# winlaic/ZipVoice

Hardware: AMD Instinct MI355X
Metric: generated mel-frames/s (whole job) + RTF, ZipVoice 123M N_steps=16 batch=32/GPU (higher is better)
Workload: dtype bf16; 1 GPU; C2: ZipVoice 123M, N_steps=16, batch=32/GPU x (3 s prompt + 10 s generated; T=1219 frames), CFG g=1.0 (64 decoder rows per GPU), t_shift=0.5; model=zipvoice (zipvoice_base.json, synthetic seeded weights), global_batch=32, seq_len=1219, parallelism=dp1

## Files before the change

### zipvoice_amd/csrc/zv_ffn.inc

```
#pragma once
#include <cstddef>
#include "zv_gemm256.inc"
#include "zv_weights.inc"

typedef unsigned v4u32_t __attribute__((ext_vector_type(4)));
typedef unsigned v2u32_t __attribute__((ext_vector_type(2)));
constexpr int FFN_D = 512, FFN_BM = 128, FFN_HC = 32, FFN_SLOT = 32768, FFN_MAXSEG = 4;
constexpr long FFN_PART_FLOATS = (long)FFN_BM * FFN_D;

struct FfnSeg {
  int M, rb0;
  const bf16* X;
  const bf16* A;
  const float* resid; float* C;
  bf16* Ch;
  const float* rowvec;
  const float* orig;
  bf16* Cl; bf16* C2h; bf16* C2l;
};

struct FfnParams {
  int H;
  int R, nseg;
  FfnSeg seg[FFN_MAXSEG];
  long ldx, ldc, ldch, rowvec_ld; int rows_per_group;
  const bf16* W1f; const float* b1;
  const bf16* W2f; const float* b2;
  const float* byp;
  const bf16* Wpf; const float* bp; long lda; int nkp;
  const float* nb; float log_scale;
  float norm_scale;
  float* sink;
  int w;
  float* part; unsigned* flag; int part_slots;
  unsigned* err;
  unsigned long long* dbg;
};

#ifndef FFN_NORM_LDS
#define FFN_NORM_LDS 1
#endif
#ifndef FFN_XOVL
#define FFN_XOVL 1
#endif
constexpr int FFN_NCONST = 3 * FFN_D + 4 * 2 * FFN_D;
inline size_t ffn_lds_bytes(int H, bool norm = false) {
  return 4 * FFN_SLOT + ((size_t)H + FFN_HC) * 4 +
         (norm && FFN_NORM_LDS ? FFN_NCONST * 4 : 0);
}

#ifdef ZV_OPERAND_F16
#define FFN_MFMA "v_mfma_f32_32x32x16_f16"
#else
#define FFN_MFMA "v_mfma_f32_32x32x16_bf16"
#endif
#ifndef FFN_BIAS_ACC
#define FFN_BIAS_ACC 1
#endif
__device__ __forceinline__ void ffn_mma_v0(f32x16& acc, const bf16x8& a, const bf16x8& b) {
  asm volatile(FFN_MFMA " %0, %1, %2, 0" : "=&v"(acc) : "v"(a), "v"(b));
}
__device__ __forceinline__ void ffn_mma_v(f32x16& acc, const bf16x8& a, const bf16x8& b) {
  asm volatile(FFN_MFMA " %0, %1, %2, %0" : "+v"(acc) : "v"(a), "v"(b));
}
#ifndef FFN_OUT_ASM
#define FFN_OUT_ASM 1
#endif
__device__ __forceinline__ void ffn_mma_a(f32x16& acc, const bf16x8& a, const bf16x8& b) {
#if FFN_OUT_ASM
  asm volatile(FFN_MFMA " %0, %1, %2, %0" : "+a"(acc) : "v"(a), "v"(b));
#else
  acc = ZV_MFMA_32x32x16(a, b, acc, 0, 0, 0);
#endif
}
struct FfnAct { float t, m, q; };
__device__ __forceinline__ void ffn_act_op(int sub, float& y, FfnAct& a, float b, float c0, float cq) {
  if (sub == 0) {
#if FFN_BIAS_ACC
    asm volatile("v_fmamk_f32 %0, %1, 0x3fb8aa3b, %2" : "=&v"(a.t) : "v"(y), "v"(c0));
#else
    asm volatile("v_add_f32 %0, %0, %2\n\tv_fmamk_f32 %1, %0, 0x3fb8aa3b, %3" : "+&v"(y), "=&v"(a.t) : "v"(b), "v"(c0));
#endif
  } else if (sub == 1) {
    asm volatile("v_min_f32 %0, 0x42fc0000, %1\n\tv_exp_f32 %0, %0" : "=&v"(a.m) : "v"(a.t));
  } else if (sub == 2) {
    asm volatile("v_add_f32 %0, 1.0, %0\n\tv_log_f32 %0, %0" : "+v"(a.m));
  } else {
    asm volatile("v_fmamk_f32 %1, %0, 0xbda3d70a, %4\n\tv_max_f32 %2, %2, %3\n\tv_fmamk_f32 %0, %2, 0x3f317218, %1"
                 : "+&v"(y), "=&v"(a.q), "+&v"(a.m) : "v"(a.t), "v"(cq));
  }
}

#ifndef FFN_DMA_K0
#define FFN_DMA_K0 1
#define FFN_DMA_K1 17
#define FFN_DMA_K2 33
#define FFN_DMA_K3 49
#endif
#ifndef FFN_TIMING
#define FFN_TIMING 0
#endif
#ifndef FFN_PD
#define FFN_PD 12
#endif
#ifndef FFN_PD_OPRE
#define FFN_PD_OPRE 8
#endif
#ifndef FFN_PD_NORM
#define FFN_PD_NORM 16
#endif
constexpr int FFN_DBG_WORDS = 10;
#ifndef FFN_X_NOACT
#define FFN_X_NOACT 0
#endif
#ifndef FFN_X_NOW1
#define FFN_X_NOW1 0
#endif
#ifndef FFN_X_NOW2
#define FFN_X_NOW2 0
#endif
#ifndef FFN_EPI_T
#define FFN_EPI_T 1
#endif
#ifndef FFN_PT
#define FFN_PT 16
#endif
#ifndef FFN_EPI_NT
#define FFN_EPI_NT 1
#endif
#ifndef FFN_PT_NORM
#define FFN_PT_NORM 8
#endif
constexpr unsigned long long FFN_SPIN_TICKS = 200000000;

template <bool RV, bool ORIG, bool COPY, int ABL = 0, int NORM = 0, bool TP = true, bool PRE = false>
__global__ __launch_bounds__(256, 1) void zv_ffn_kernel(FfnParams p) {
  extern __shared__ __attribute__((aligned(16))) unsigned char smem[];
  const int tid = threadIdx.x, lane = tid & 63;
  const int wave = __builtin_amdgcn_readfirstlane(tid >> 6);
  const int tl = lane & 31, hh = lane >> 5;
  const int nc = p.H / FFN_HC;
  float* b1s = reinterpret_cast<float*>(smem + 4 * FFN_SLOT);
  const long Wtot = (long)p.R * nc;
  const long start = (long)blockIdx.x * p.w;
  if (start >= Wtot) return;
  const long end = min(start + (long)p.w, Wtot);

  auto dma = [&](const bf16* W, int c, int slot, int half) {
    const unsigned long long a = (unsigned long long)W + (unsigned long long)((long)c * FFN_SLOT + wave * 8192 + half * 4096);
    const unsigned long long b =
        ((unsigned long long)(unsigned)__builtin_amdgcn_readfirstlane((unsigned)(a >> 32)) << 32) |
        (unsigned long long)(unsigned)__builtin_amdgcn_readfirstlane((unsigned)a);
    glds16s_x4(reinterpret_cast<const void*>(b), (unsigned)lane * 16u, smem + slot * FFN_SLOT + wave * 8192 + half * 4096);
  };
  auto item_at = [&](long ps, int& r, int& ca, int& cb) {
    r = (int)(ps / nc);
    const int c = (int)(ps - (long)r * nc);
    if (c != 0) { ca = 0; cb = nc - c; }
    else if (ps + nc <= end) { ca = 0; cb = nc; }
    else { ca = nc - (int)(end - ps); cb = nc; }
  };

  int r, ca, cb;
  item_at(start, r, ca, cb);
  dma(p.W1f, ca, 0, 0); dma(p.W1f, ca, 0, 1);
  dma(p.W1f, ca + 1, 1, 0); dma(p.W1f, ca + 1, 1, 1);
  for (int i = tid; i < p.H + FFN_HC; i += 256) b1s[i] = i < p.H ? p.b1[i] : 0.f;
  constexpr bool NLDS = NORM && FFN_NORM_LDS;
  float* ncs = b1s + p.H + FFN_HC;
  if constexpr (NLDS) {
    for (int i = tid; i < FFN_D; i += 256) {
      ncs[i] = p.b2[i];
      ncs[FFN_D + i] = p.nb[i];
      ncs[2 * FFN_D + i] = p.byp[i];
    }
  }

  float c0 = -5.77078016355585362f, cq = -0.035f;
  asm volatile("" : "+v"(c0), "+v"(cq));
  const int lfrag = lane * 16;
  int lfrag2 = lane * 16 + 2 * FFN_SLOT;
  asm volatile("" : "+v"(lfrag2));
  auto w1f = [&](int sl, int s) { return *reinterpret_cast<const bf16x8*>(smem + sl * FFN_SLOT + s * 1024 + lfrag); };
  auto w2f = [&](int sl, int i) { return *reinterpret_cast<const bf16x8*>(smem + sl * FFN_SLOT + i * 1024 + lfrag2); };
  auto put = [&](bf16x8 (&hb)[2], int rr, float y) { hb[rr >> 3][rr & 7] = (bf16)y; };
  const __amdgpu_buffer_rsrc_t part_rs = __builtin_amdgcn_make_buffer_rsrc(p.part, 0, 0x7fffffff, 0x00020000);

#if FFN_TIMING
  unsigned long long tm_vm = 0, tm_bar = 0, tm_steps = 0, tm_epi = 0, tm_x = 0, tm_items = 0, tm_loop = 0;
  const unsigned long long tm_t0 = __builtin_amdgcn_s_memtime(), tm_r0 = __builtin_amdgcn_s_memrealtime();
#endif
  auto item = [&](auto KIND_, int r, int ca, int cb, bool has_next, int nca) {
    constexpr int KIND = decltype(KIND_)::value;
    constexpr bool split_in = KIND == 2, split_out = KIND == 1;
    const int nxt_c0 = has_next ? nca : cb - 1;
    const int nxt_c1 = has_next ? nca + 1 : cb - 1;
    f32x16 out[16];
    int sg = 0;
#pragma unroll
    for (int i = 1; i < FFN_MAXSEG; ++i) sg = (i < p.nseg && r >= p.seg[i].rb0) ? i : sg;
    typedef __attribute__((address_space(4))) const FfnSeg KSeg;
    KSeg& S = ((KSeg*)((__attribute__((address_space(4))) const char*)__builtin_amdgcn_kernarg_segment_ptr() +
                       offsetof(FfnParams, seg)))[sg];
    const int t0 = (r - S.rb0) * FFN_BM + wave * 32;

    if constexpr (split_in) {
      if (tid == 0) {
        GLOBAL unsigned* fl = (GLOBAL unsigned*)(p.flag + blockIdx.x + 1);
        const unsigned long long t_give_up = wall_clock64() + FFN_SPIN_TICKS;
        while (__hip_atomic_load(fl, __ATOMIC_RELAXED, __HIP_MEMORY_SCOPE_AGENT) == 0u) {
          __builtin_amdgcn_s_sleep(2);
          if (wall_clock64() > t_give_up) {
            if (p.err) __hip_atomic_store(p.err, 1u, __ATOMIC_RELAXED, __HIP_MEMORY_SCOPE_SYSTEM);
            break;
          }
        }
        __builtin_amdgcn_fence(__ATOMIC_ACQUIRE, "agent");
        __hip_atomic_store(fl, 0u, __ATOMIC_RELAXED, __HIP_MEMORY_SCOPE_AGENT);
      }
      asm volatile("s_waitcnt vmcnt(0)" ::: "memory");
      __syncthreads();
      int lv = lane;
      asm volatile("" : "+v"(lv));
      const f32x4* src = reinterpret_cast<const f32x4*>(p.part + (long)(blockIdx.x + 1) * FFN_PART_FLOATS) + wave * 4096 + lv;
      static_for<16>([&](auto J_) {
        constexpr int j = decltype(J_)::value;
        f32x4 v[4];
#pragma unroll
        for (int q = 0; q < 4; ++q) v[q] = src[(j * 4 + q) * 64];
        out[j] = f32x16{v[0][0], v[0][1], v[0][2], v[0][3], v[1][0], v[1][1], v[1][2], v[1][3],
                        v[2][0], v[2][1], v[2][2], v[2][3], v[3][0], v[3][1], v[3][2], v[3][3]};
        __builtin_amdgcn_sched_barrier(0);
      });
    } else if constexpr (!PRE) {
#pragma unroll
      for (int j = 0; j < 16; ++j) out[j] = f32x16{};
    }
    if constexpr (!PRE || split_in) {
#pragma unroll
      for (int j = 0; j < 16; ++j) asm volatile("" : "+a"(out[j]));
    }
#if FFN_TIMING
    const unsigned long long tx0 = __builtin_amdgcn_s_memtime();
    ++tm_items;
#endif
    const bool nrv = NLDS && !split_out && S.rowvec != nullptr && p.rows_per_group >= 32;
    const int nrv_g0 = nrv ? min(t0, S.M - 1) / p.rows_per_group : 0;
    f32x4 nrvv[4];
    if constexpr (NLDS && !split_out) {
      if (nrv) {
        const int g1 = min(nrv_g0 + 1, (S.M - 1) / p.rows_per_group);
#pragma unroll
        for (int q = 0; q < 4; ++q) {
          const int f = (q * 64 + lane) * 4;
          const int grp = f < FFN_D ? nrv_g0 : g1;
          nrvv[q] = *reinterpret_cast<const f32x4*>(S.rowvec + (long)grp * p.rowvec_ld + (f & (FFN_D - 1)));
        }
      }
    }
    bf16x8 xf[32];
    if constexpr (!PRE) {
      const int tr = min(t0 + tl, S.M - 1);
      const bf16* xr = S.X + (long)tr * p.ldx + 8 * hh;
#pragma unroll
      for (int s = 0; s < 32; ++s) xf[s] = *reinterpret_cast<const bf16x8*>(xr + 16 * s);
    } else if constexpr (split_in) {
      const int tr = min(t0 + tl, S.M - 1);
      const bf16* xr = S.Ch + (long)tr * p.ldch + 4 * hh;
#pragma unroll
      for (int s = 0; s < 32; ++s) {
        const bf16x4 lo = *reinterpret_cast<const bf16x4*>(xr + 16 * s), hi = *reinterpret_cast<const bf16x4*>(xr + 16 * s + 8);
        xf[s] = bf16x8{lo[0], lo[1], lo[2], lo[3], hi[0], hi[1], hi[2], hi[3]};
      }
    }
    wait_vmcnt<(FFN_XOVL && !PRE) ? 32 : 0>();
    if constexpr (NLDS && !split_out) {
      if (nrv) {
#pragma unroll
        for (int q = 0; q < 4; ++q)
          *reinterpret_cast<f32x4*>(ncs + 3 * FFN_D + wave * 2 * FFN_D + (q * 64 + lane) * 4) = nrvv[q];
      }
    }
    __syncthreads();
#if FFN_TIMING
    tm_x += __builtin_amdgcn_s_memtime() - tx0;
#endif

    if constexpr (PRE && !split_in) {
      int lvp = lane;
      asm volatile("" : "+v"(lvp));
      const int ptl = lvp & 31, phh = lvp >> 5;
      const int wr = max(0, min(32, S.M - t0));
      const __amdgpu_buffer_rsrc_t rs_a =
          __builtin_amdgcn_make_buffer_rsrc(const_cast<bf16*>(S.A + (long)t0 * p.lda), 0, wr * (int)p.lda * 2, 0x00020000);
      const __amdgpu_buffer_rsrc_t rs_pr =
          __builtin_amdgcn_make_buffer_rsrc(const_cast<float*>(S.resid + (long)t0 * p.ldc), 0, wr * (int)p.ldc * 4, 0x00020000);
      const int a_off = (ptl * (int)p.lda + 8 * phh) * 2, r_off = (ptl * (int)p.ldc + 4 * phh) * 4;
      auto load_a = [&](int kc, int s) {
        return __builtin_bit_cast(bf16x8, __builtin_amdgcn_raw_buffer_load_b128(rs_a, a_off + kc * 64 + s * 32, 0, 0));
      };
      dma(p.Wpf, 0, 2, 0); dma(p.Wpf, 0, 2, 1);
      bf16x8 ac[2], an[2];
      ac[0] = load_a(0, 0); ac[1] = load_a(0, 1);
      const bool hrv = S.rowvec != nullptr;
      const int rpg = hrv ? p.rows_per_group : 1;
      auto tile_of = [&](const f32x4 (&v)[4]) {
        return f32x16{v[0][0], v[0][1], v[0][2], v[0][3], v[1][0], v[1][1], v[1][2], v[1][3],
                      v[2][0], v[2][1], v[2][2], v[2][3], v[3][0], v[3][1], v[3][2], v[3][3]};
      };
      if (!hrv || rpg >= 32) {
        float* cvs = reinterpret_cast<float*>(smem + 3 * FFN_SLOT) + wave * 2 * FFN_D;
        const int g0 = hrv ? min(t0, S.M - 1) / rpg : 0;
        const int g1 = hrv ? min(g0 + 1, (S.M - 1) / rpg) : 0;
#pragma unroll
        for (int q = 0; q < 4; ++q) {
          const int f = (q * 64 + lvp) * 4, ch = f & (FFN_D - 1);
          f32x4 v = *reinterpret_cast<const f32x4*>(p.bp + ch);
          if (hrv) v += *reinterpret_cast<const f32x4*>(S.rowvec + (long)(f < FFN_D ? g0 : g1) * p.rowvec_ld + ch);
          *reinterpret_cast<f32x4*>(cvs + f) = v;
        }
        asm volatile("s_waitcnt lgkmcnt(0)" ::: "memory");
        __builtin_amdgcn_wave_barrier();
        const float* cvp = cvs + ((hrv && t0 + ptl >= (g0 + 1) * rpg) ? FFN_D : 0) + 4 * phh;
        constexpr int PDT = 6;
        f32x4 ri[16][4];
        auto pf = [&](int j) {
          if (j < 16) {
#pragma unroll
            for (int q = 0; q < 4; ++q)
              ri[j][q] = __builtin_bit_cast(f32x4, __builtin_amdgcn_raw_buffer_load_b128(rs_pr, r_off + (32 * j + 8 * q) * 4, 0, 0));
          }
        };
#pragma unroll
        for (int j = 0; j < PDT; ++j) pf(j);
        static_for<16>([&](auto J_) {
          constexpr int j = decltype(J_)::value;
          pf(j + PDT);
          f32x4 v[4];
#pragma unroll
          for (int q = 0; q < 4; ++q) v[q] = ri[j][q] + *reinterpret_cast<const f32x4*>(cvp + 32 * j + 8 * q);
          out[j] = tile_of(v);
          asm volatile("" : "+a"(out[j]));
          __builtin_amdgcn_sched_barrier(0);
        });
      } else {
        const int grp = min(t0 + ptl, S.M - 1) / rpg;
        const float* vrow = S.rowvec + (long)grp * p.rowvec_ld + 4 * phh;
        const float* bpl = p.bp + 4 * phh;
        static_for<16>([&](auto J_) {
          constexpr int j = decltype(J_)::value;
          f32x4 v[4];
#pragma unroll
          for (int q = 0; q < 4; ++q) {
            const f32x4 r4 = __builtin_bit_cast(f32x4, __builtin_amdgcn_raw_buffer_load_b128(rs_pr, r_off + (32 * j + 8 * q) * 4, 0, 0));
            v[q] = r4 + (*reinterpret_cast<const f32x4*>(bpl + 32 * j + 8 * q) + *reinterpret_cast<const f32x4*>(vrow + 32 * j + 8 * q));
          }
          out[j] = tile_of(v);
          asm volatile("" : "+a"(out[j]));
          if constexpr ((j & 3) == 3) __builtin_amdgcn_sched_barrier(0);
        });
      }
      auto pstep = [&](auto PAR_, int kc) {
        constexpr int PAR = decltype(PAR_)::value;
        wait_vmcnt<0>();
        asm volatile("s_waitcnt lgkmcnt(0)" ::: "memory");
        __builtin_amdgcn_s_barrier();
        asm volatile("s_nop 7\n\ts_nop 7\n\ts_nop 3" ::: "memory");
        if (kc + 1 < p.nkp) { dma(p.Wpf, kc + 1, 3 - PAR, 0); dma(p.Wpf, kc + 1, 3 - PAR, 1); }
        const int kn = min(kc + 1, p.nkp - 1);
        an[0] = load_a(kn, 0); an[1] = load_a(kn, 1);
        bf16x8 fb[4];
#pragma unroll
        for (int q = 0; q < 4; ++q) fb[q] = w2f(PAR, q);
        static_for<32>([&](auto I_) {
          constexpr int i = decltype(I_)::value;
          ffn_mma_a(out[i >> 1], fb[i & 3], ac[i & 1]);
          if constexpr (i + 4 < 32) fb[i & 3] = w2f(PAR, i + 4);
        });
        asm volatile("" ::"v"(ac[0]), "v"(ac[1]), "v"(fb[0]), "v"(fb[1]), "v"(fb[2]), "v"(fb[3]));
        ac[0] = an[0]; ac[1] = an[1];
      };
      int kc = 0;
      for (; kc + 1 < p.nkp; kc += 2) {
        pstep(std::integral_constant<int, 0>{}, kc);
        pstep(std::integral_constant<int, 1>{}, kc + 1);
      }
      if (kc < p.nkp) pstep(std::integral_constant<int, 0>{}, kc);
      asm volatile("s_nop 7\n\ts_nop 7\n\ts_nop 3" ::: "memory");
#pragma unroll
      for (int j = 0; j < 16; ++j) asm volatile("" : "+a"(out[j]));
      static_for<32>([&](auto S_) {
        constexpr int s = decltype(S_)::value, jt = s >> 1, pp = s & 1;
#pragma unroll
        for (int e = 0; e < 8; ++e) xf[s][e] = (bf16)out[jt][8 * pp + e];
      });
#pragma unroll
      for (int j = 0; j < 16; ++j) asm volatile("" : "+a"(out[j]));
      if constexpr (split_out) {
        const __amdgpu_buffer_rsrc_t rs_xh =
            __builtin_amdgcn_make_buffer_rsrc(S.Ch + (long)t0 * p.ldch, 0, wr * (int)p.ldch * 2, 0x00020000);
        const int h_off = (ptl * (int)p.ldch + 4 * phh) * 2;
        static_for<32>([&](auto S_) {
          constexpr int s = decltype(S_)::value;
          const v4u32_t w = __builtin_bit_cast(v4u32_t, xf[s]);
          __builtin_amdgcn_raw_buffer_store_b64(v2u32_t{w[0], w[1]}, rs_xh, h_off + 32 * s, 0, 16);
          __builtin_amdgcn_raw_buffer_store_b64(v2u32_t{w[2], w[3]}, rs_xh, h_off + 32 * s + 16, 0, 16);
        });
      }
#pragma unroll
      for (int s = 0; s < 32; ++s) asm volatile("" : "+v"(xf[s]));
      asm volatile("s_nop 7\n\ts_nop 7\n\ts_nop 3" ::: "memory");
    }

    auto bias4 = [&](int c, int q) { return *reinterpret_cast<const f32x4*>(b1s + c * FFN_HC + 8 * q + 4 * hh); };
    auto bias_tile = [&](int c) {
      const f32x4 q0 = bias4(c, 0), q1 = bias4(c, 1), q2 = bias4(c, 2), q3 = bias4(c, 3);
      return f32x16{q0[0], q0[1], q0[2], q0[3], q1[0], q1[1], q1[2], q1[3],
                    q2[0], q2[1], q2[2], q2[3], q3[0], q3[1], q3[2], q3[3]};
    };
    f32x16 h0, h1;
#if FFN_BIAS_ACC
    h0 = bias_tile(ca);
    h1 = bias_tile(ca + 1);
#endif
    {
      bf16x8 f[4];
#pragma unroll
      for (int q = 0; q < 4; ++q) f[q] = w1f(0, q);
      static_for<32>([&](auto S_) {
        constexpr int s = decltype(S_)::value;
        if constexpr (s == 0 && !FFN_BIAS_ACC) ffn_mma_v0(h0, f[0], xf[0]);
        else ffn_mma_v(h0, f[s & 3], xf[s]);
        if constexpr (s + 4 < 32) f[s & 3] = w1f(0, s + 4);
      });
    }
    asm volatile("s_nop 7\n\ts_nop 7\n\ts_nop 3" : "+v"(h0));
    __builtin_amdgcn_s_barrier();

    auto sync = [&]() {
#if FFN_TIMING
      const unsigned long long ts0 = __builtin_amdgcn_s_memtime();
#endif
      wait_vmcnt<0>();
      asm volatile("s_waitcnt lgkmcnt(0)" ::: "memory");
#if FFN_TIMING
      const unsigned long long ts1 = __builtin_amdgcn_s_memtime();
#endif
      __builtin_amdgcn_s_barrier();
#if FFN_TIMING
      const unsigned long long ts2 = __builtin_amdgcn_s_memtime();
      tm_vm += ts1 - ts0;
      tm_bar += ts2 - ts1;
      ++tm_steps;
#endif
      asm volatile("s_nop 7\n\ts_nop 7\n\ts_nop 3" ::: "memory");
    };
    auto w1_next = [&](int c) { return c + 2 <= cb - 1 ? c + 2 : (c + 2 == cb ? nxt_c0 : nxt_c1); };

    bf16x8 hb0[2], hb1[2];
    {
      const int c1 = w1_next(ca);
      dma(p.W1f, c1, 0, 0); dma(p.W1f, c1, 0, 1);
      dma(p.W2f, ca, 2, 0); dma(p.W2f, ca, 2, 1);
      f32x4 bq = FFN_BIAS_ACC ? f32x4{} : bias4(ca, 0);
      FfnAct a{};
      bf16x8 f[4];
#pragma unroll
      for (int q = 0; q < 4; ++q) f[q] = w1f(1, q);
      static_for<32>([&](auto S_) {
        constexpr int s = decltype(S_)::value, rr = s >> 1;
        if constexpr (s == 0 && !FFN_BIAS_ACC) ffn_mma_v0(h1, f[0], xf[0]);
        else ffn_mma_v(h1, f[s & 3], xf[s]);
        if constexpr (s + 4 < 32) f[s & 3] = w1f(1, s + 4);
        if constexpr ((rr & 3) == 0 && (s & 1) == 0 && !FFN_BIAS_ACC) bq = bias4(ca, rr >> 2);
        float y = h0[rr];
        ffn_act_op(2 * (s & 1), y, a, bq[rr & 3], c0, cq);
        ffn_act_op(2 * (s & 1) + 1, y, a, bq[rr & 3], c0, cq);
        h0[rr] = y;
        if constexpr (s & 1) put(hb0, rr, y);
      });
#if FFN_BIAS_ACC
      h0 = bias_tile(min(ca + 2, nc));
#endif
      asm volatile("s_nop 7\n\ts_nop 7\n\ts_nop 3" : "+v"(h1));
      sync();
      asm volatile("" ::"v"(f[0]), "v"(f[1]), "v"(f[2]), "v"(f[3]));
    }

    const int m = t0 + tl;
    const bool row_ok = m < S.M;
    const long mr = min(m, S.M - 1);
    const float* rrow = S.resid + mr * p.ldc;
    const float* orow = (ORIG || NORM) ? S.orig + mr * p.ldc : nullptr;
    constexpr bool OPRE = ORIG && !NORM;
    constexpr int PD = NORM ? FFN_PD_NORM : OPRE ? FFN_PD_OPRE : FFN_PD;
    f32x4 rr[32][2], ro[OPRE ? 32 : 1][2];
    auto prefetch = [&](int g) {
      if (g < 32) {
        const int n = 16 * g + 8 * hh;
        if constexpr (!PRE) {
          rr[g][0] = *reinterpret_cast<const f32x4*>(rrow + n);
          rr[g][1] = *reinterpret_cast<const f32x4*>(rrow + n + 4);
        }
        if constexpr (OPRE) {
          ro[g][0] = *reinterpret_cast<const f32x4*>(orow + n);
          ro[g][1] = *reinterpret_cast<const f32x4*>(orow + n + 4);
        }
      }
    };

    constexpr bool EPT = FFN_EPI_T && TP && !NORM && ABL != 3;
    constexpr bool EPN = FFN_EPI_NT && TP && NORM && NLDS && ABL != 3 && !split_out;
    constexpr bool TORIG = EPT && ORIG;
    constexpr int PT = NORM ? FFN_PT_NORM : FFN_PT;
    int lve = lane;
    asm volatile("" : "+v"(lve));
    const int lr = lve >> 5, lc = lve & 31, ltl = lve & 31, lhh = lve >> 5;
    const int wrows = max(0, min(32, S.M - t0));
    f32x4 tq[EPT ? 64 : EPN ? 128 : 1], to[TORIG ? 64 : 1];
    const __amdgpu_buffer_rsrc_t rs_r =
        __builtin_amdgcn_make_buffer_rsrc(const_cast<float*>(S.resid + (long)t0 * p.ldc), 0, wrows * (int)p.ldc * 4, 0x00020000);
    const __amdgpu_buffer_rsrc_t rs_o = __builtin_amdgcn_make_buffer_rsrc(
        (TORIG || EPN) ? const_cast<float*>(S.orig + (long)t0 * p.ldc) : p.sink, 0,
        (TORIG || EPN) ? wrows * (int)p.ldc * 4 : 0, 0x00020000);
    const int toff = (lr * (int)p.ldc + 4 * lc) * 4, tstep = 2 * (int)p.ldc * 4;
    const bool has_rv = EPT && RV;
    const bool rv_two = has_rv && p.rows_per_group >= 32;
    const int rv_g0 = has_rv ? min(t0, S.M - 1) / p.rows_per_group : 0;
    const int rv_g1 = has_rv ? min(rv_g0 + 1, (S.M - 1) / p.rows_per_group) : 0;
    const int rv_bnd = has_rv ? (rv_g0 + 1) * p.rows_per_group - t0 : 0;
    constexpr bool TCONST = EPT && !ORIG;
    f32x4 cb2[TCONST ? 4 : 1], cby[TCONST ? 4 : 1], crv0[TCONST ? 4 : 1], crv1[TCONST ? 4 : 1];
    auto load_consts = [&]() {
      if constexpr (TCONST) {
#pragma unroll
        for (int ps = 0; ps < 4; ++ps) {
          const int col = ps * 128 + 4 * lc;
          if constexpr (EPT) cb2[ps] = *reinterpret_cast<const f32x4*>(p.b2 + col);
          if constexpr (TORIG) cby[ps] = *reinterpret_cast<const f32x4*>(p.byp + col);
          if (rv_two) {
// ... 348 lines not shown
            const f32x4 w0 = *reinterpret_cast<const f32x4*>(ncs + vl_off + n);
            const f32x4 w1 = *reinterpret_cast<const f32x4*>(ncs + vl_off + n + 4);
#pragma unroll
            for (int e = 0; e < 4; ++e) { y[e] += w0[e]; y[4 + e] += w1[e]; }
          } else if (vrow) {
            const f32x4 w0 = *reinterpret_cast<const f32x4*>(vrow + n);
            const f32x4 w1 = *reinterpret_cast<const f32x4*>(vrow + n + 4);
#pragma unroll
            for (int e = 0; e < 4; ++e) { y[e] += w0[e]; y[4 + e] += w1[e]; }
          }
#pragma unroll
          for (int e = 0; e < 8; ++e) { h[e] = (bf16)y[e]; l[e] = (bf16)(y[e] - (float)h[e]); }
          if (row_ok) {
            *reinterpret_cast<bf16x8*>(C2hp + oh) = h;
            if (C2lp) *reinterpret_cast<bf16x8*>(C2lp + oh) = l;
          }
        }
      });
    } else if constexpr (EPT) {
      __builtin_amdgcn_s_barrier();
      float* tb = reinterpret_cast<float*>(smem + 2 * FFN_SLOT) + wave * 4096;
      const __amdgpu_buffer_rsrc_t rs_c = __builtin_amdgcn_make_buffer_rsrc(Cp + (long)t0 * p.ldc, 0, wrows * (int)p.ldc * 4, 0x00020000);
      const __amdgpu_buffer_rsrc_t rs_h =
          __builtin_amdgcn_make_buffer_rsrc(COPY ? (void*)(Chp + (long)t0 * p.ldch) : (void*)p.sink, 0, COPY ? wrows * (int)p.ldch * 2 : 0, 0x00020000);
      const int hoff = (lr * (int)p.ldch + 4 * lc) * 2, hstep = 2 * (int)p.ldch * 2;
      static_for<4>([&](auto P_) {
        constexpr int ps = decltype(P_)::value;
        static_for<4>([&](auto J_) {
          constexpr int jj = decltype(J_)::value, j = 4 * ps + jj;
#pragma unroll
          for (int q = 0; q < 4; ++q) {
            const int ch = (8 * jj + 2 * q + lhh) ^ (ltl & 7);
            *reinterpret_cast<f32x4*>(tb + ltl * 128 + ch * 4) =
                f32x4{out[j][4 * q], out[j][4 * q + 1], out[j][4 * q + 2], out[j][4 * q + 3]};
          }
        });
        __builtin_amdgcn_sched_barrier(0);
        const int col = ps * 128 + 4 * lc;
        f32x4 bb, sc4{};
        if constexpr (TCONST) bb = cb2[ps];
        else {
          bb = *reinterpret_cast<const f32x4*>(p.b2 + col);
          if constexpr (ORIG) sc4 = *reinterpret_cast<const f32x4*>(p.byp + col);
        }
        const f32x4 rv0 = crv0[ps], rv1 = crv1[ps];
        static_for<16>([&](auto I_) {
          constexpr int i = decltype(I_)::value, k = 16 * ps + i;
          tprefetch(k + PT);
          const int row = 2 * i + lr;
          const f32x4 a = *reinterpret_cast<const f32x4*>(tb + row * 128 + ((lc ^ (row & 7)) * 4));
          f32x4 v;
#pragma unroll
          for (int e = 0; e < 4; ++e) v[e] = PRE ? a[e] + bb[e] : tq[k][e] + (a[e] + bb[e]);
          const int mrow = t0 + row;
          if constexpr (RV) {
            const bool second = row >= rv_bnd;
            f32x4 w;
#pragma unroll
            for (int e = 0; e < 4; ++e) w[e] = second ? rv1[e] : rv0[e];
#pragma unroll
            for (int e = 0; e < 4; ++e) v[e] += w[e];
          }
          if constexpr (ORIG) {
#pragma unroll
            for (int e = 0; e < 4; ++e)
              v[e] = PRE ? __builtin_fmaf(v[e] - to[k][e], sc4[e], to[k][e]) : to[k][e] + (v[e] - to[k][e]) * sc4[e];
          }
          __builtin_amdgcn_raw_buffer_store_b128(__builtin_bit_cast(v4u32_t, v), rs_c, toff + i * tstep + ps * 512, 0, 0);
          if constexpr (COPY) {
            bf16x4 h;
#pragma unroll
            for (int e = 0; e < 4; ++e) h[e] = (bf16)v[e];
            __builtin_amdgcn_raw_buffer_store_b64(__builtin_bit_cast(v2u32_t, h), rs_h, hoff + i * hstep + ps * 256, 0, 0);
          }
          __builtin_amdgcn_sched_barrier(0);
        });
      });
    } else {
      const float* vrow = RV ? S.rowvec + (mr / p.rows_per_group) * p.rowvec_ld : nullptr;
      static_for<32>([&](auto G_) {
        constexpr int g = decltype(G_)::value, j = g >> 1, pp = g & 1;
        prefetch(g + PD);
        const int n = 16 * g + 8 * hh;
        float v[8];
#pragma unroll
        for (int e = 0; e < 4; ++e) {
          const auto sw = __builtin_amdgcn_permlane32_swap(__float_as_uint(out[j][8 * pp + e]),
                                                           __float_as_uint(out[j][8 * pp + 4 + e]), false, false);
          v[e] = __uint_as_float(sw[0]);
          v[4 + e] = __uint_as_float(sw[1]);
        }
        const f32x4 b0 = *reinterpret_cast<const f32x4*>(p.b2 + n);
        const f32x4 b1 = *reinterpret_cast<const f32x4*>(p.b2 + n + 4);
#pragma unroll
        for (int e = 0; e < 4; ++e) {
          v[e] = PRE ? v[e] + b0[e] : rr[g][0][e] + (v[e] + b0[e]);
          v[4 + e] = PRE ? v[4 + e] + b1[e] : rr[g][1][e] + (v[4 + e] + b1[e]);
        }
        if constexpr (RV) {
          const f32x4 w0 = *reinterpret_cast<const f32x4*>(vrow + n);
          const f32x4 w1 = *reinterpret_cast<const f32x4*>(vrow + n + 4);
#pragma unroll
          for (int e = 0; e < 4; ++e) { v[e] += w0[e]; v[4 + e] += w1[e]; }
        }
        if constexpr (ORIG) {
          const f32x4 s0 = *reinterpret_cast<const f32x4*>(p.byp + n);
          const f32x4 s1 = *reinterpret_cast<const f32x4*>(p.byp + n + 4);
#pragma unroll
          for (int e = 0; e < 4; ++e) {
            v[e] = ro[g][0][e] + (v[e] - ro[g][0][e]) * s0[e];
            v[4 + e] = ro[g][1][e] + (v[4 + e] - ro[g][1][e]) * s1[e];
          }
        }
        unsigned long long cadr = c_base + (unsigned long long)(n * c_mul);
        asm volatile("" : "+v"(cadr));
        *(GLOBAL f32x4*)(cadr) = f32x4{v[0], v[1], v[2], v[3]};
        *(GLOBAL f32x4*)(cadr + 16) = f32x4{v[4], v[5], v[6], v[7]};
        if constexpr (COPY) {
          bf16x8 h;
#pragma unroll
          for (int e = 0; e < 8; ++e) h[e] = (bf16)v[e];
          unsigned long long ha2 = h_base + (unsigned long long)(n * h_mul);
          asm volatile("" : "+v"(ha2));
          *(GLOBAL bf16x8*)(ha2) = h;
        }
      });
    }
#if FFN_TIMING
    asm volatile("s_waitcnt vmcnt(0)" ::: "memory");
    tm_epi += __builtin_amdgcn_s_memtime() - te0;
#endif
  };

  long pos = start;
  for (;;) {
    const bool split_in = ca > 0, split_out = cb < nc;
    const long npos = split_out ? (long)(r + 1) * nc : (split_in ? end : pos + nc);
    const bool has_next = npos < end;
    int nr = 0, nca = 0, ncb = 0;
    if (has_next) item_at(npos, nr, nca, ncb);
    if (split_out) item(std::integral_constant<int, 1>{}, r, ca, cb, has_next, nca);
    else if (split_in) item(std::integral_constant<int, 2>{}, r, ca, cb, has_next, nca);
    else item(std::integral_constant<int, 0>{}, r, ca, cb, has_next, nca);
    if (!has_next) break;
    pos = npos; r = nr; ca = nca; cb = ncb;
  }
#if FFN_TIMING
  if (lane == 0) {
    unsigned long long* d = p.dbg + ((long)blockIdx.x * 4 + wave) * FFN_DBG_WORDS;
    d[0] = __builtin_amdgcn_s_memtime() - tm_t0;
    d[1] = __builtin_amdgcn_s_memrealtime() - tm_r0;
    d[2] = tm_vm; d[3] = tm_bar; d[4] = tm_steps; d[5] = (unsigned long long)p.w;
    d[6] = tm_epi; d[7] = tm_x; d[8] = tm_items; d[9] = tm_loop;
  }
#endif
}

static __global__ void zv_ffn_pack_w1_kernel(const bf16* W, long ldw, int H, bf16* out) {
  const long i = blockIdx.x * 256L + threadIdx.x;
  if (i >= (long)H * FFN_D) return;
  const int j = (int)(i & 7);
  long r = i >> 3;
  const int l = (int)(r & 63); r >>= 6;
  const int s = (int)(r & 31), c = (int)(r >> 5);
  out[i] = W[(long)(32 * c + (l & 31)) * ldw + 16 * s + 8 * (l >> 5) + j];
}
static __global__ void zv_ffn_pack_w2_kernel(const bf16* W, long ldw, int H, bf16* out) {
  const long i = blockIdx.x * 256L + threadIdx.x;
  if (i >= (long)H * FFN_D) return;
  const int j = (int)(i & 7);
  long r = i >> 3;
  const int l = (int)(r & 63); r >>= 6;
  const int s = (int)(r & 1); r >>= 1;
  const int jb = (int)(r & 15), c = (int)(r >> 4);
  out[i] = W[(long)(32 * jb + (l & 31)) * ldw + 32 * c + 16 * s + 8 * (j >> 2) + 4 * (l >> 5) + (j & 3)];
}
static __global__ void zv_ffn_pack_w1p_kernel(const bf16* W, long ldw, int H, bf16* out) {
  const long i = blockIdx.x * 256L + threadIdx.x;
  if (i >= (long)H * FFN_D) return;
  const int j = (int)(i & 7);
  long r = i >> 3;
  const int l = (int)(r & 63); r >>= 6;
  const int s = (int)(r & 31), c = (int)(r >> 5);
  out[i] = W[(long)(32 * c + (l & 31)) * ldw + 16 * s + 8 * (j >> 2) + 4 * (l >> 5) + (j & 3)];
}
static __global__ void zv_ffn_pack_wp_kernel(const bf16* W, long ldw, int K, int nkp, bf16* out) {
  const long i = blockIdx.x * 256L + threadIdx.x;
  if (i >= (long)nkp * FFN_HC * FFN_D) return;
  const int j = (int)(i & 7);
  long r = i >> 3;
  const int l = (int)(r & 63); r >>= 6;
  const int s = (int)(r & 1); r >>= 1;
  const int jb = (int)(r & 15), kc = (int)(r >> 4);
  const int k = 32 * kc + 16 * s + 8 * (l >> 5) + j;
  out[i] = k < K ? W[(long)(32 * jb + (l & 31)) * ldw + k] : (bf16)0.f;
}
inline int ffn_pre_chunks(int K) { return (K + FFN_HC - 1) / FFN_HC; }
static void ffn_pack_pre_weights(const Linear& L1, int H, bf16* w1fp, const Linear& Lp, bf16* wpf, hipStream_t s) {
  const long n = (long)H * FFN_D, np = (long)ffn_pre_chunks(Lp.K) * FFN_HC * FFN_D;
  hipLaunchKernelGGL(zv_ffn_pack_w1p_kernel, dim3(cdiv(n, 256)), dim3(256), 0, s, L1.hi, (long)L1.Kpad, H, w1fp);
  hipLaunchKernelGGL(zv_ffn_pack_wp_kernel, dim3(cdiv(np, 256)), dim3(256), 0, s, Lp.hi, (long)Lp.Kpad, Lp.K,
                     ffn_pre_chunks(Lp.K), wpf);
  ZV_LAUNCH_CHECK();
}
static void ffn_pack_weights(const Linear& L1, const Linear& L2, int H, bf16* w1f, bf16* w2f, hipStream_t s) {
  const long n = (long)H * FFN_D;
  hipLaunchKernelGGL(zv_ffn_pack_w1_kernel, dim3(cdiv(n, 256)), dim3(256), 0, s, L1.hi, (long)L1.Kpad, H, w1f);
  hipLaunchKernelGGL(zv_ffn_pack_w2_kernel, dim3(cdiv(n, 256)), dim3(256), 0, s, L2.hi, (long)L2.Kpad, H, w2f);
  ZV_LAUNCH_CHECK();
}

struct FfnSchedule { int w, blocks; };
inline FfnSchedule ffn_schedule(int R, int nc, int blocks_max, bool persistent) {
  if (!persistent || R <= blocks_max) return {nc, R};
  const long W = (long)R * nc;
  long w = (W + blocks_max - 1) / blocks_max;
  w = std::max<long>(round_up(w, 2), nc);
  return {(int)w, (int)((W + w - 1) / w)};
}

template <bool RV, bool ORIG, bool COPY, int ABL = 0, int NORM = 0, bool TP = true, bool PRE = false>
static void launch_ffn_t(const FfnParams& p, int blocks, hipStream_t s, const char* tag) {
  static unsigned long long attr = 0;
  const size_t lds = ffn_lds_bytes(p.H, NORM != 0);
  if (!((attr >> zv_cur_device()) & 1)) {
    ZV_CHECK(hipFuncSetAttribute((const void*)zv_ffn_kernel<RV, ORIG, COPY, ABL, NORM, TP, PRE>,
                                 hipFuncAttributeMaxDynamicSharedMemorySize, 160 * 1024));
    attr |= 1ull << zv_cur_device();
  }
  double M = 0, extra = 0;
  for (int i = 0; i < p.nseg; ++i) {
    const FfnSeg& g = p.seg[i];
    M += g.M;
    if (NORM) extra += (double)g.M * FFN_D * ((g.Cl ? 2 : 0) + (g.C2h ? 2 : 0) + (g.C2l ? 2 : 0));
  }
  const double outs = M * FFN_D;
  const double Kp = PRE ? (double)p.nkp * FFN_HC : 0.0;
  const double bytes = (PRE ? (M + FFN_D) * Kp * 2 : outs * 2) + 2.0 * FFN_D * p.H * 2 +
                       (NORM ? outs * (4 + 4 + 4 + 2) + extra : outs * (8 + (COPY ? 2 : 0) + (ORIG ? 4 : 0)));
  g_zv_last_launch = ZvLaunchRec{FFN_BM, FFN_D, 1, (int)RV | (int)ORIG << 1 | (int)COPY << 2 | (int)TP << 3 | (int)PRE << 4, NORM,
                                 0, blocks, p.w};
  ZvProfScope prof(tag, 4.0 * M * FFN_D * (double)p.H + 2.0 * M * FFN_D * Kp, bytes, s);
  hipLaunchKernelGGL((zv_ffn_kernel<RV, ORIG, COPY, ABL, NORM, TP, PRE>), dim3(blocks), dim3(256), lds, s, p);
  ZV_LAUNCH_CHECK();
}

template <int ABL = 0>
static void launch_ffn(FfnParams p, hipStream_t s, const char* tag, int blocks_max = 0) {
  ZV_REQUIRE(p.H > 0 && p.H % (2 * FFN_HC) == 0 && ffn_lds_bytes(p.H, p.nb != nullptr) <= 160 * 1024,
             "fused FeedForward: hidden width a multiple of 64 (LDS: at most 8160, 2496 with the BiasNorm epilogue)");
  ZV_REQUIRE(p.nseg >= 1 && p.nseg <= FFN_MAXSEG, "fused FeedForward: 1..4 row ranges");
  ZV_REQUIRE(p.W1f && p.W2f && p.b1 && p.b2 && (p.Wpf || (p.ldx % 8 == 0 && p.ldx >= FFN_D)) && p.ldc % 4 == 0 &&
                 p.ldc >= FFN_D && (p.ldch == 0 || (p.ldch % 8 == 0 && p.ldch >= FFN_D)),
             "fused FeedForward operands (16-B aligned rows of at least 512)");
  const bool rv = p.seg[0].rowvec != nullptr, og = p.seg[0].orig != nullptr, cp = p.seg[0].Ch != nullptr;
  const bool pre = p.Wpf != nullptr;
  ZV_REQUIRE(!pre || (p.bp && p.nkp >= 1 && p.lda >= (long)p.nkp * FFN_HC && p.lda % 8 == 0 && cp && og),
             "fused FeedForward pre-projection operands (lda >= Kp, 16-B aligned rows, the bypass or BiasNorm site)");
  int R = 0;
  for (int i = 0; i < p.nseg; ++i) {
    FfnSeg& g = p.seg[i];
    ZV_REQUIRE(!pre || g.A, "fused FeedForward pre-projection operand");
    ZV_REQUIRE(g.M > 0 && (g.X || pre) && g.resid && g.C && (g.Ch != nullptr) == cp && (g.rowvec != nullptr) == rv &&
                   (g.orig != nullptr) == og && (!g.Ch || p.ldch > 0),
               "fused FeedForward row range operands");
    g.rb0 = R;
    R += cdiv(g.M, FFN_BM);
  }
  ZV_REQUIRE(og == (p.byp != nullptr) && (!rv || p.rows_per_group > 0), "fused FeedForward bypass / row vector");
  p.R = R;
  p.sink = zv_epi_sink();
  p.err = zv_dev_err_word();
  const int nc = p.H / FFN_HC;
  const bool pers = p.part && p.flag;
  int bmax = blocks_max > 0 ? std::min(blocks_max, zv_num_cus()) : zv_num_cus();
  if (pers) {
    ZV_REQUIRE(p.part_slots > 0, "fused FeedForward: persistent scratch without its slot count");
    bmax = std::min(bmax, p.part_slots);
  }
  const FfnSchedule sc = ffn_schedule(R, nc, bmax, pers);
  ZV_REQUIRE(!pers || sc.w == nc || sc.blocks <= bmax, "fused FeedForward: more lines than scratch slots");
  p.w = sc.w;
  if (p.nb) {
    for (int i = 0; i < p.nseg; ++i)
      ZV_REQUIRE(p.seg[i].orig && p.seg[i].C == p.seg[i].orig && p.seg[i].Ch,
                 "fused FeedForward + BiasNorm operands");
    ZV_REQUIRE(p.byp, "fused FeedForward + BiasNorm bypass");
    p.norm_scale = expf(p.log_scale);
    const bool tp = !(p.seg[0].rowvec && p.rows_per_group < 32);
    if (pre) {
      if (tp) launch_ffn_t<false, false, true, 0, 1, true, true>(p, sc.blocks, s, tag);
      else launch_ffn_t<false, false, true, 0, 1, false, true>(p, sc.blocks, s, tag);
    } else if (tp) launch_ffn_t<false, false, true, 0, 1>(p, sc.blocks, s, tag);
    else launch_ffn_t<false, false, true, 0, 1, false>(p, sc.blocks, s, tag);
    return;
  }
  if constexpr (ABL != 0) { launch_ffn_t<false, false, true, ABL>(p, sc.blocks, s, tag); return; }
  if (pre) {
    ZV_REQUIRE(og && cp, "fused FeedForward pre-projection: the bypass site");
    launch_ffn_t<false, true, true, 0, 0, true, true>(p, sc.blocks, s, tag);
    return;
  }
  if (!rv && !og && cp) launch_ffn_t<false, false, true>(p, sc.blocks, s, tag);
  else if (!rv && !og && !cp) launch_ffn_t<false, false, false>(p, sc.blocks, s, tag);
  else if (rv && !og && cp) {
    if (p.rows_per_group >= 32) launch_ffn_t<true, false, true>(p, sc.blocks, s, tag);
// ... 6 lines not shown
```

Baseline: 87310 mel-frames/s.

## Stream residual loads into the projection K-loop instead of prefetching upfront

The pre-projection path used to load all 16 residual tiles into registers before the GEMM K-loop and add them into the accumulator initialisation. Now the accumulators start from bias/rowvec only, and the residual tiles are loaded in groups interleaved with the K-steps, then added to the accumulators one step later. This hides residual load latency behind MFMA work. Buffer resources are also made wave-uniform via readfirstlane, and extra timing counters are added under FFN_TIMING. The risks are more register pressure from in-flight loads and a dependence on nkp being at least NG+1 steps.

```diff
diff --git a/zipvoice_amd/csrc/zv_ffn.inc b/zipvoice_amd/csrc/zv_ffn.inc
--- a/zipvoice_amd/csrc/zv_ffn.inc
+++ b/zipvoice_amd/csrc/zv_ffn.inc
@@ -43,7 +43,10 @@
 #ifndef FFN_XOVL
 #define FFN_XOVL 1
 #endif
-constexpr int FFN_NCONST = 3 * FFN_D + 4 * 2 * FFN_D;
+#ifndef FFN_PRE_NT
+#define FFN_PRE_NT 1
+#endif
+constexpr int FFN_NCONST =3 * FFN_D + 4 * 2 * FFN_D;
 inline size_t ffn_lds_bytes(int H, bool norm = false) {
   return 4 * FFN_SLOT + ((size_t)H + FFN_HC) * 4 +
          (norm && FFN_NORM_LDS ? FFN_NCONST * 4 : 0);
@@ -109,7 +112,7 @@
 #ifndef FFN_PD_NORM
 #define FFN_PD_NORM 16
 #endif
-constexpr int FFN_DBG_WORDS = 10;
+constexpr int FFN_DBG_WORDS = 15;
 #ifndef FFN_X_NOACT
 #define FFN_X_NOACT 0
 #endif
@@ -188,6 +191,7 @@
 
 #if FFN_TIMING
   unsigned long long tm_vm = 0, tm_bar = 0, tm_steps = 0, tm_epi = 0, tm_x = 0, tm_items = 0, tm_loop = 0;
+  unsigned long long tm_pinit = 0, tm_ploop = 0, tm_pvm = 0, tm_pbar = 0, tm_psteps = 0;
   const unsigned long long tm_t0 = __builtin_amdgcn_s_memtime(), tm_r0 = __builtin_amdgcn_s_memrealtime();
 #endif
   auto item = [&](auto KIND_, int r, int ca, int cb, bool has_next, int nca) {
@@ -291,14 +295,22 @@
       asm volatile("" : "+v"(lvp));
       const int ptl = lvp & 31, phh = lvp >> 5;
       const int wr = max(0, min(32, S.M - t0));
-      const __amdgpu_buffer_rsrc_t rs_a =
-          __builtin_amdgcn_make_buffer_rsrc(const_cast<bf16*>(S.A + (long)t0 * p.lda), 0, wr * (int)p.lda * 2, 0x00020000);
-      const __amdgpu_buffer_rsrc_t rs_pr =
-          __builtin_amdgcn_make_buffer_rsrc(const_cast<float*>(S.resid + (long)t0 * p.ldc), 0, wr * (int)p.ldc * 4, 0x00020000);
+      auto uniform_rsrc = [&](const void* base, int bytes) {
+        const unsigned long long a = (unsigned long long)base;
+        const unsigned long long b =
+            ((unsigned long long)(unsigned)__builtin_amdgcn_readfirstlane((unsigned)(a >> 32)) << 32) |
+            (unsigned long long)(unsigned)__builtin_amdgcn_readfirstlane((unsigned)a);
+        return __builtin_amdgcn_make_buffer_rsrc(reinterpret_cast<void*>(b), 0, __builtin_amdgcn_readfirstlane(bytes), 0x00020000);
+      };
+      const __amdgpu_buffer_rsrc_t rs_a = uniform_rsrc(S.A + (long)t0 * p.lda, wr * (int)p.lda * 2);
+      const __amdgpu_buffer_rsrc_t rs_pr = uniform_rsrc(S.resid + (long)t0 * p.ldc, wr * (int)p.ldc * 4);
       const int a_off = (ptl * (int)p.lda + 8 * phh) * 2, r_off = (ptl * (int)p.ldc + 4 * phh) * 4;
       auto load_a = [&](int kc, int s) {
         return __builtin_bit_cast(bf16x8, __builtin_amdgcn_raw_buffer_load_b128(rs_a, a_off + kc * 64 + s * 32, 0, 0));
       };
+#if FFN_TIMING
+      const unsigned long long tp0 = __builtin_amdgcn_s_memtime();
+#endif
       dma(p.Wpf, 0, 2, 0); dma(p.Wpf, 0, 2, 1);
       bf16x8 ac[2], an[2];
       ac[0] = load_a(0, 0); ac[1] = load_a(0, 1);
@@ -322,26 +334,14 @@
         asm volatile("s_waitcnt lgkmcnt(0)" ::: "memory");
         __builtin_amdgcn_wave_barrier();
         const float* cvp = cvs + ((hrv && t0 + ptl >= (g0 + 1) * rpg) ? FFN_D : 0) + 4 * phh;
-        constexpr int PDT = 6;
-        f32x4 ri[16][4];
-        auto pf = [&](int j) {
-          if (j < 16) {
-#pragma unroll
-            for (int q = 0; q < 4; ++q)
-              ri[j][q] = __builtin_bit_cast(f32x4, __builtin_amdgcn_raw_buffer_load_b128(rs_pr, r_off + (32 * j + 8 * q) * 4, 0, 0));
-          }
-        };
-#pragma unroll
-        for (int j = 0; j < PDT; ++j) pf(j);
         static_for<16>([&](auto J_) {
           constexpr int j = decltype(J_)::value;
-          pf(j + PDT);
           f32x4 v[4];
 #pragma unroll
-          for (int q = 0; q < 4; ++q) v[q] = ri[j][q] + *reinterpret_cast<const f32x4*>(cvp + 32 * j + 8 * q);
+          for (int q = 0; q < 4; ++q) v[q] = *reinterpret_cast<const f32x4*>(cvp + 32 * j + 8 * q);
           out[j] = tile_of(v);
           asm volatile("" : "+a"(out[j]));
-          __builtin_amdgcn_sched_barrier(0);
+          if constexpr ((j & 3) == 3) __builtin_amdgcn_sched_barrier(0);
         });
       } else {
         const int grp = min(t0 + ptl, S.M - 1) / rpg;
@@ -351,41 +351,93 @@
           constexpr int j = decltype(J_)::value;
           f32x4 v[4];
 #pragma unroll
-          for (int q = 0; q < 4; ++q) {
-            const f32x4 r4 = __builtin_bit_cast(f32x4, __builtin_amdgcn_raw_buffer_load_b128(rs_pr, r_off + (32 * j + 8 * q) * 4, 0, 0));
-            v[q] = r4 + (*reinterpret_cast<const f32x4*>(bpl + 32 * j + 8 * q) + *reinterpret_cast<const f32x4*>(vrow + 32 * j + 8 * q));
-          }
+          for (int q = 0; q < 4; ++q)
+            v[q] = *reinterpret_cast<const f32x4*>(bpl + 32 * j + 8 * q) + *reinterpret_cast<const f32x4*>(vrow + 32 * j + 8 * q);
           out[j] = tile_of(v);
           asm volatile("" : "+a"(out[j]));
           if constexpr ((j & 3) == 3) __builtin_amdgcn_sched_barrier(0);
         });
       }
-      auto pstep = [&](auto PAR_, int kc) {
-        constexpr int PAR = decltype(PAR_)::value;
-        wait_vmcnt<0>();
+      constexpr int NT = FFN_PRE_NT, NG = 16 / NT;
+      static_assert(NT >= 1 && NT * NG == 16, "FFN_PRE_NT divides the 16 tiles");
+      f32x4 ri[16][4];
+      auto rload = [&](auto G_) {
+        constexpr int g = decltype(G_)::value;
+        if constexpr (g >= 0 && g < NG) {
+#pragma unroll
+          for (int j = g * NT; j < (g + 1) * NT; ++j) {
+#pragma unroll
+            for (int q = 0; q < 4; ++q)
+              ri[j][q] = __builtin_bit_cast(f32x4, __builtin_amdgcn_raw_buffer_load_b128(rs_pr, r_off + (32 * j + 8 * q) * 4, 0, 0));
+          }
+        }
+      };
+      auto radd = [&](auto G_) {
+        constexpr int g = decltype(G_)::value;
+        if constexpr (g >= 0 && g < NG) {
+          static_for<NT>([&](auto T_) {
+            constexpr int j = g * NT + decltype(T_)::value;
+            asm volatile("" : "+a"(out[j]));
+            out[j] += tile_of(ri[j]);
+            asm volatile("" : "+a"(out[j]));
+          });
+        }
+      };
+      rload(std::integral_constant<int, 0>{});
+#if FFN_TIMING
+      const unsigned long long tp1 = __builtin_amdgcn_s_memtime();
+      tm_pinit += tp1 - tp0;
+#endif
+      auto pstep = [&](auto KC_, int kc) {
+        constexpr int KC = decltype(KC_)::value;
+        int nk = p.nkp;
+        asm volatile("" : "+s"(nk));
+        const int sl = min(kc, nk - 1) & 1;
+        const bool nx = kc + 1 < nk;
+        const int n_so = nx ? (kc + 1) * 64 : 0x40000000;
+#if FFN_TIMING
+        const unsigned long long ts0 = __builtin_amdgcn_s_memtime();
+#endif
+        wait_vmcnt<(KC >= 0 && KC < NG) ? 4 * NT : 0>();
         asm volatile("s_waitcnt lgkmcnt(0)" ::: "memory");
+#if FFN_TIMING
+        const unsigned long long ts1 = __builtin_amdgcn_s_memtime();
+#endif
         __builtin_amdgcn_s_barrier();
+#if FFN_TIMING
+        tm_pvm += ts1 - ts0;
+        tm_pbar += __builtin_amdgcn_s_memtime() - ts1;
+        ++tm_psteps;
+#endif
         asm volatile("s_nop 7\n\ts_nop 7\n\ts_nop 3" ::: "memory");
-        if (kc + 1 < p.nkp) { dma(p.Wpf, kc + 1, 3 - PAR, 0); dma(p.Wpf, kc + 1, 3 - PAR, 1); }
-        const int kn = min(kc + 1, p.nkp - 1);
-        an[0] = load_a(kn, 0); an[1] = load_a(kn, 1);
+        if constexpr (KC >= 1) {
+          radd(std::integral_constant<int, KC - 1>{});
+          asm volatile("s_nop 3" ::: "memory");
+        }
+        if (nx) { dma(p.Wpf, kc + 1, 3 - sl, 0); dma(p.Wpf, kc + 1, 3 - sl, 1); }
+        const int n_off = a_off + n_so;
+        an[0] = __builtin_bit_cast(bf16x8, __builtin_amdgcn_raw_buffer_load_b128(rs_a, n_off, 0, 0));
+        an[1] = __builtin_bit_cast(bf16x8, __builtin_amdgcn_raw_buffer_load_b128(rs_a, n_off + 32, 0, 0));
+        if constexpr (KC >= 0) rload(std::integral_constant<int, KC + 1>{});
+        int fbase = lfrag2 + sl * FFN_SLOT;
+        asm volatile("" : "+v"(fbase));
+        auto wpf = [&](int i) { return *reinterpret_cast<const bf16x8*>(smem + i * 1024 + fbase); };
         bf16x8 fb[4];
 #pragma unroll
-        for (int q = 0; q < 4; ++q) fb[q] = w2f(PAR, q);
+        for (int q = 0; q < 4; ++q) fb[q] = wpf(q);
         static_for<32>([&](auto I_) {
           constexpr int i = decltype(I_)::value;
           ffn_mma_a(out[i >> 1], fb[i & 3], ac[i & 1]);
-          if constexpr (i + 4 < 32) fb[i & 3] = w2f(PAR, i + 4);
+          if constexpr (i + 4 < 32) fb[i & 3] = wpf(i + 4);
         });
         asm volatile("" ::"v"(ac[0]), "v"(ac[1]), "v"(fb[0]), "v"(fb[1]), "v"(fb[2]), "v"(fb[3]));
         ac[0] = an[0]; ac[1] = an[1];
       };
-      int kc = 0;
-      for (; kc + 1 < p.nkp; kc += 2) {
-        pstep(std::integral_constant<int, 0>{}, kc);
-        pstep(std::integral_constant<int, 1>{}, kc + 1);
-      }
-      if (kc < p.nkp) pstep(std::integral_constant<int, 0>{}, kc);
+      static_for<NG + 1>([&](auto KC_) { pstep(KC_, decltype(KC_)::value); });
+      for (int kc = NG + 1; kc < p.nkp; ++kc) pstep(std::integral_constant<int, -1>{}, kc);
+#if FFN_TIMING
+      tm_ploop += __builtin_amdgcn_s_memtime() - tp1;
+#endif
       asm volatile("s_nop 7\n\ts_nop 7\n\ts_nop 3" ::: "memory");
 #pragma unroll
       for (int j = 0; j < 16; ++j) asm volatile("" : "+a"(out[j]));
@@ -1040,6 +1092,7 @@
     d[1] = __builtin_amdgcn_s_memrealtime() - tm_r0;
     d[2] = tm_vm; d[3] = tm_bar; d[4] = tm_steps; d[5] = (unsigned long long)p.w;
     d[6] = tm_epi; d[7] = tm_x; d[8] = tm_items; d[9] = tm_loop;
+    d[10] = tm_pinit; d[11] = tm_ploop; d[12] = tm_pvm; d[13] = tm_pbar; d[14] = tm_psteps;
   }
 #endif
 }
```

Result: no change. 87990 mel-frames/s, median of 6 (+0.8%).
